# jgsimard/big-dreamer

Measured on AMD Instinct MI355X. Metric: latent transitions/sec (RSSM + imagination) at batch=50 chunk=50 H=15, higher is better.
Workload: dtype f32

## Files before the change

big_dreamer_amd/_cabi.py:

```python
from __future__ import annotations

import ctypes as C
import os

import torch

_HERE = os.path.dirname(os.path.abspath(__file__))
LIB_PATH = os.environ.get("BD_LIB") or os.path.join(_HERE, "libbigdreamer_hip.so")

if not os.path.exists(LIB_PATH):
    raise ImportError(
        f"{LIB_PATH} is missing: the MI355X HIP extension has not been built "
        "(run `python -c 'import __graft_entry__ as g; g.build()'`). There is no CPU fallback.")

lib = C.CDLL(LIB_PATH)

BD_MAX_LAYERS = 6
ACT_NONE, ACT_ELU, ACT_ELU_GRAD = 0, 1, 2
P = C.c_void_p
F32 = C.c_float
I32 = C.c_int


class PackDesc(C.Structure):
    _fields_ = [("src", P), ("dst", P), ("ld", I32), ("N", I32), ("K", I32), ("transpose", I32)]


class Layer(C.Structure):
    _fields_ = [("w", P), ("bias", P), ("N", I32), ("K", I32), ("act", I32), ("save", P)]


class MlpFwdArgs(C.Structure):
    _fields_ = [("M", I32), ("in0", P), ("ld0", I32), ("w0", I32), ("in1", P), ("ld1", I32), ("w1", I32),
                ("n_layers", I32), ("layer", Layer * BD_MAX_LAYERS), ("out", P), ("ldo", I32),
                ("gidx", P), ("gWT", P), ("gD", I32), ("gC", I32)]


class LayerBwd(C.Structure):
    _fields_ = [("wt", P), ("saved", P), ("N", I32), ("K", I32), ("act", I32), ("dpre", P)]


class MlpBwdArgs(C.Structure):
    _fields_ = [("M", I32), ("dout", P), ("lddo", I32), ("dout_scale", F32), ("n_layers", I32),
                ("layer", LayerBwd * BD_MAX_LAYERS), ("din0", P), ("ld0", I32), ("w0", I32),
                ("din1", P), ("ld1", I32), ("w1", I32), ("accumulate", I32)]


BD_RNG_MAX_TENSORS = 6
BD_RNG_NORMAL, BD_RNG_EXPONENTIAL = 0, 1


class RngTensor(C.Structure):
    _fields_ = [("p", P), ("count", C.c_size_t), ("kind", I32), ("stream_id", C.c_uint)]


class RngFillArgs(C.Structure):
    _fields_ = [("n", I32), ("seed", C.c_ulonglong), ("step", C.c_ulonglong), ("t", RngTensor * BD_RNG_MAX_TENSORS)]


class WgradDesc(C.Structure):
    _fields_ = [("dpre", P), ("ldp", I32), ("act1", P), ("lda1", I32), ("M1", I32), ("act2", P), ("lda2", I32),
                ("M", I32), ("N", I32), ("K", I32), ("dW", P), ("ldw", I32), ("db", P),
                ("splits", I32), ("rows_per", I32), ("tiles_n", I32), ("tiles_k", I32), ("block_begin", I32),
                ("red_begin", I32), ("ws_off", C.c_ulonglong),
                ("g_nseg", I32), ("g_seglen", I32), ("g_gh", I32), ("g_gw", I32), ("g_IH", I32), ("g_IW", I32), ("g_C", I32),
                ("g_pad", I32)]


def _ptr_fields(names):
    return [(n, P) for n in names]


class ObserveFwdArgs(C.Structure):
    _fields_ = ([(n, I32) for n in ("T", "B", "Be", "S", "A", "Hd")] + _ptr_fields(
        ["w_embed_s", "w_embed_a", "b_embed", "w_ir", "w_iz", "w_in", "w_hr", "w_hz", "w_hn", "b_ih", "b_hh",
         "w_q1h", "b_q1", "w_q2m", "w_q2s", "b_q2", "init_belief", "init_state", "actions", "nonterm", "pre_emb",
         "eps_post"]) + [("min_std", F32)] + _ptr_fields(
        ["feat", "post_mean", "post_std", "sv_s", "sv_x", "sv_gates", "sv_q"]))


class ObserveBwdArgs(C.Structure):
    _fields_ = ([(n, I32) for n in ("T", "B", "Be", "S", "A", "Hd")] + _ptr_fields(
        ["wt_embed_s", "wt_ir", "wt_iz", "wt_in", "wt_hr", "wt_hz", "wt_hn", "wt_q1h", "wt_q2m", "wt_q2s",
         "init_belief", "nonterm", "eps_post", "feat", "post_std", "sv_x", "sv_gates", "sv_q", "dfeat", "dpost_mean",
         "dpost_std"]) + [("min_std", F32)] + _ptr_fields(
        ["d_embed_pre", "d_gi", "d_gh", "d_q1_pre", "d_q2_out"]))


class ImagineFwdArgs(C.Structure):
    _fields_ = ([(n, I32) for n in ("N", "Hm", "Be", "S", "A", "Hd", "n_samples")] + _ptr_fields(
        ["w_embed_s", "w_embed_a", "b_embed", "w_ir", "w_iz", "w_in", "w_hr", "w_hz", "w_hn", "b_ih", "b_hh", "w_p1",
         "b_p1", "w_p2m", "w_p2s", "b_p2", "w_a0h", "w_a0s"]) + [("w_a", P * 3), ("b_a", P * 4)] + _ptr_fields(
        ["w_a4m", "w_a4s", "b_a4", "start_feat", "eps_action", "eps_entropy", "eps_prior"]) + [
        ("min_std", F32), ("act_raw_init_std", F32), ("act_min_std", F32), ("act_mean_scale", F32)] + _ptr_fields(
        ["feat", "prior_mean", "prior_std", "entropy", "action", "sv_actor", "sv_act_stats", "sv_x", "sv_gates",
         "sv_p"]) + [("sv_actor_stride", C.c_size_t)] + _ptr_fields(["sv_act_us"]) + [("discrete_actions", I32)])


# ... 57 lines not shown
                ("OH", I32), ("OW", I32), ("osy", I32), ("oy0", I32), ("osx", I32), ("ox0", I32), ("ldo", I32),
                ("act", I32), ("fuse_cq", I32), ("aux", P)]


_SIGS = {
    "bd_last_error": (C.c_char_p, []),
    "bd_version": (I32, []),
    "bd_packed_floats": (C.c_size_t, [I32, I32]),
    "bd_pack_weights": (I32, [P, I32, P]),
    "bd_mlp_forward": (I32, [C.POINTER(MlpFwdArgs), P]),
    "bd_mlp_backward": (I32, [C.POINTER(MlpBwdArgs), P]),
    "bd_mlp_set_tall": (I32, [I32]),
    "bd_wgrad_ws_floats": (C.c_size_t, [I32, I32, I32]),
    "bd_wgrad": (I32, [P, I32, P, I32, I32, I32, I32, P, I32, P, I32, P, C.c_size_t, P]),
    "bd_wgrad_plan": (I32, [C.POINTER(WgradDesc), I32, C.POINTER(I32), C.POINTER(I32), C.POINTER(C.c_size_t)]),
    "bd_wgrad_grouped": (I32, [P, I32, I32, I32, P, P]),
    "bd_wgrad_grouped_phase": (I32, [P, I32, I32, I32, P, I32, P]),
    "bd_observe_forward": (I32, [C.POINTER(ObserveFwdArgs), P]),
    "bd_observe_backward": (I32, [C.POINTER(ObserveBwdArgs), P]),
    "bd_observe_cluster_size": (I32, [I32, I32]),
    "bd_observe_cluster_ws_floats": (C.c_size_t, [I32, I32]),
    "bd_observe_forward_cluster": (I32, [C.POINTER(ObserveFwdArgs), P, C.c_size_t, P]),
    "bd_observe_backward_cluster": (I32, [C.POINTER(ObserveBwdArgs), P, C.c_size_t, P]),
    "bd_observe_cluster_status": (I32, [P, I32, P]),
    "bd_observe_cluster_err_offset": (C.c_size_t, [I32]),
    "bd_observe_cluster_set_spin_limit": (I32, [C.c_uint]),
    "bd_observe_cluster_set_ksplit": (I32, [I32]),
    "bd_gauss_head_forward": (I32, [P, P, I32, I32, F32, P, P, P, P]),
    "bd_gauss_head_backward": (I32, [P, P, P, P, P, I32, I32, P, P]),
    "bd_observe_cat_forward": (I32, [C.POINTER(ObserveCatFwdArgs), P]),
    "bd_observe_cat_backward": (I32, [C.POINTER(ObserveCatBwdArgs), P]),
    "bd_observe_cat_cluster_size": (I32, [I32, I32, I32, I32, I32]),
    "bd_observe_cat_cluster_ws_floats": (C.c_size_t, [I32, I32, I32, I32, I32]),
    "bd_observe_cat_forward_cluster": (I32, [C.POINTER(ObserveCatFwdArgs), I32, P, C.c_size_t, P]),
    "bd_observe_cat_backward_cluster": (I32, [C.POINTER(ObserveCatBwdArgs), I32, P, C.c_size_t, P]),
    "bd_imagine_cat_forward": (I32, [C.POINTER(ImagineCatFwdArgs), P]),
    "bd_imagine_cat_backward": (I32, [C.POINTER(ImagineCatBwdArgs), P]),
    "bd_imagine_forward": (I32, [C.POINTER(ImagineFwdArgs), P]),
    "bd_imagine_forward_scan": (I32, [C.POINTER(ImagineFwdArgs), P]),
    "bd_actor_entropy": (I32, [P, P, P, I32, I32, I32, I32, P]),
    "bd_imagine_backward": (I32, [C.POINTER(ImagineBwdArgs), P]),
    "bd_lambda_return_forward": (I32, [P, P, I32, I32, F32, F32, P, P]),
    "bd_rng_fill": (I32, [C.POINTER(RngFillArgs), P]),
    "bd_philox4x32_10": (I32, [C.POINTER(C.c_uint), C.POINTER(C.c_uint), C.POINTER(C.c_uint)]),
    "bd_actor_entropy_rng": (I32, [C.c_ulonglong, C.c_ulonglong, C.c_uint, P, P, I32, I32, I32, I32, P]),
    "bd_gemm_nt": (I32, [P, I32, P, I32, P, I32, I32, I32, I32, I32, P]),
    "bd_categorical_head_forward": (I32, [P, P, I32, I32, I32, P, P, P]),
    "bd_categorical_head_backward": (I32, [P, P, I32, I32, I32, P, P]),
    "bd_kl_categorical_forward": (I32, [P, P, I32, I32, I32, F32, I32, P, I32, P, P]),
    "bd_kl_categorical_backward": (I32, [P, P, I32, I32, I32, F32, F32, F32, F32, P, I32, P, P, P]),
    "bd_plan_rollout": (I32, [C.POINTER(PlanArgs), P]),
    "bd_cem_refit": (I32, [P, I32, P, I32, I32, I32, I32, I32, P, P, P]),
    "bd_lambda_return_backward": (I32, [P, F32, I32, I32, F32, F32, P, P, P]),
    "bd_actor_reinforce": (I32, [P, P, P, P, P, P, P, I32, I32, I32, F32, F32, F32, I32, P, P, I32, P, P]),
    "bd_actor_reinforce_cat": (I32, [P, P, P, P, P, P, I32, I32, I32, F32, F32, F32, I32, P, P, I32, P, P]),
    "bd_normal_nll": (I32, [P, I32, P, I32, I32, I32, F32, P, I32, P, I32, P, P]),
    "bd_bernoulli_nll": (I32, [P, P, C.c_size_t, F32, P, P, I32, P, P]),
    "bd_kl_forward": (I32, [P, P, P, P, I32, I32, F32, I32, P, I32, P, P]),
    "bd_kl_backward": (I32, [P, P, P, P, I32, I32, F32, F32, F32, F32, P, I32, P, P, P, P, P]),
    "bd_sum": (I32, [P, C.c_size_t, P, I32, P, P]),
    "bd_sumsq": (I32, [P, C.c_size_t, P, I32, P, P]),
    "bd_adam_step": (I32, [P, P, P, P, C.c_size_t, F32, F32, F32, F32, F32, I32, F32, P, I32, P]),
    "bd_polyak": (I32, [P, P, C.c_size_t, F32, P]),
    "bd_replay_gather": (I32, [P, P, I32, I32, P, P]),
    "bd_replay_gather_pixels": (I32, [P, P, I32, I32, I32, P, P, P]),
    "bd_replay_gather_pixels_rng": (I32, [P, P, I32, I32, I32, C.c_ulonglong, C.c_ulonglong, P, P]),
    "bd_reduce_ws_floats": (C.c_size_t, []),
    "bd_conv_gemm": (I32, [C.POINTER(ConvArgs), P]),
    "bd_conv_thin_forward": (I32, [P, I32, I32, I32, I32, I32, P, I32, P, I32, P, P, P]),
    "bd_conv_pack_class": (I32, [P, P, I32, I32, I32, I32, I32, I32, I32, P]),
    "bd_conv_pack_fused": (I32, [P, P, I32, I32, I32, P]),
    "bd_elu_backward": (I32, [P, P, C.c_size_t, P]),
    "bd_image_layout": (I32, [P, P, I32, I32, I32, I32, P]),
    "bd_colsum_ws_floats": (C.c_size_t, [I32]),
    "bd_colsum": (I32, [P, C.c_size_t, I32, P, P, P]),
}

for _name, (_res, _args) in _SIGS.items():
    _fn = getattr(lib, _name)
    _fn.restype = _res
    _fn.argtypes = _args

EXPORTED = tuple(_SIGS)


def check(rc: int) -> None:
    if rc != 0:
        raise RuntimeError("bigdreamer_hip: " + lib.bd_last_error().decode())


def ptr(t) -> int:
    if t is None:
        return None
    if not (t.dtype in (torch.float32, torch.int64, torch.uint8) and t.is_cuda):
        raise TypeError("expected a CUDA fp32/int64/uint8 tensor")
    if not (t.is_contiguous() or (t.dim() == 2 and t.stride(1) == 1 and t.stride(0) >= t.shape[1])):
        raise ValueError(f"non-contiguous tensor (shape {tuple(t.shape)}, strides {t.stride()}) passed to a HIP kernel: "
                         "call .contiguous() first")
    return t.data_ptr()


def stream() -> int:
    return torch.cuda.current_stream().cuda_stream


def packed_floats(N: int, K: int) -> int:
# ... 2 lines not shown
```

big_dreamer_amd/engine.py:

```python
from __future__ import annotations

import collections.abc
import ctypes as C
import math
import os
import weakref
from typing import Dict, List, Optional, Tuple

import numpy as np
import torch

from . import _cabi as cabi
from .parallel import DataParallel
from .synth import DENSE_LAYERS, MODEL_MODULES, Dims, model_modules, param_shapes

lib = cabi.lib
ptr = cabi.ptr

DEFAULT_HP = dict(
    kl_balance=0.8, kl_loss_weight=0.1, free_nats=3.0, grad_clip_norm=100.0, discount=0.995, disclam=0.95,
    model_learning_rate=2e-4, actor_learning_rate=4e-5, value_learning_rate=1e-4, adam_epsilon=1e-5,
    weight_decay=1e-6, entropy_weight=1e-5, polyak_avg=1.0, min_std_dev=0.1, discount_weight=5.0,
    gradient_mixing=-1,
)
# ... 208 lines not shown

class DreamerEngine:
    def __init__(self, dims: Dims, hp: Optional[dict] = None, device="cuda", params: Optional[dict] = None,
                 world_size: int = 1, process_group=None, phase_groups: Optional[dict] = None):
        self.d = dims
        self.pixel = bool(dims.pixel)
        self.hp = dict(DEFAULT_HP)
        if hp:
            self.hp.update({k: v for k, v in hp.items() if k in self.hp})
        self.hp["gradient_mixing"] = check_gradient_mixing(self.hp["gradient_mixing"])
        self.dev = torch.device(device)
        assert self.dev.type == "cuda", "the HIP path needs a GPU (there is no CPU fallback)"
        self.world_size = world_size
        self.pg = process_group
        rehearsal = os.environ.get("BD_FORCE_DP", "0") == "1" and torch.distributed.is_initialized()
        if (phase_groups is None and (world_size > 1 or rehearsal) and os.environ.get("BD_PHASE_GROUPS", "1") != "0"
                and torch.distributed.get_backend(process_group) == "nccl"):
            phase_groups = DataParallel.make_phase_groups("nccl", process_group)
        self.dp = DataParallel(world_size, torch.distributed.get_rank(process_group) if world_size > 1 else 0,
                               process_group, phase_groups)
        if (world_size > 1 or rehearsal) and torch.distributed.get_backend(process_group) == "nccl":
            self.dp.force = self.dp.force or rehearsal
            tiny = torch.zeros(4, dtype=torch.float32, device=self.dev)
            for g in (None, "model", "actor", "critic"):
                self.dp.allreduce_sum_(tiny, g)
            torch.cuda.synchronize(self.dev)
        d = dims
        shapes = param_shapes(d)
        self.groups = {
            "model": ParamGroup([(m, n, s) for m in model_modules(d) for n, s in shapes[m]], self.dev,
                                conv_storage=self.pixel),
            "actor": ParamGroup([("actor", n, s) for n, s in shapes["actor"]], self.dev),
            "critic": ParamGroup([("critic", n, s) for n, s in shapes["critic"]], self.dev),
            "critic_target": ParamGroup([("critic_target", n, s) for n, s in shapes["critic"]], self.dev, False),
        }
        self._mod_group = {m: "model" for m in model_modules(d)}
        self._mod_group.update(actor="actor", critic="critic", critic_target="critic_target")
        if params is not None:
            self.load_params(params)
        self.scalars = torch.zeros(N_SLOTS, dtype=torch.float32, device=self.dev)
        self.red_ws = torch.zeros(int(lib.bd_reduce_ws_floats()), dtype=torch.float32, device=self.dev)
        self._wgrad_ws = torch.zeros(1, dtype=torch.float32, device=self.dev)
        self._wgrad_ws_side = torch.zeros(1, dtype=torch.float32, device=self.dev)
        self._wgrad_ws_early = torch.zeros(1, dtype=torch.float32, device=self.dev)
        self.red_ws_side = torch.zeros(int(lib.bd_reduce_ws_floats()), dtype=torch.float32, device=self.dev)
        self._wbatch = {"model": WgradBatch(self, "model"), "model_early": WgradBatch(self, "model_early", "_wgrad_ws_early"),
                        "actor": WgradBatch(self, "actor", "_wgrad_ws_bh"),
                        "critic": WgradBatch(self, "critic", "_wgrad_ws_side")}
        self.overlap_critic = os.environ.get("BD_OVERLAP_CRITIC", "0") == "1"
        self._side = _engine_stream(self.dev, "side", int(os.environ.get("BD_SIDE_PRIO", "0")))
        self._s_heads = _engine_stream(self.dev, "heads", -1)
        self.img_split = os.environ.get("BD_IMG_SPLIT", "0") == "1"
        self._img_split_rows = 0
        self._s_early = _engine_stream(self.dev, "early", int(os.environ.get("BD_EARLY_PRIO", "0")))
        self.pipeline = os.environ.get("BD_PIPELINE", "1") != "0"
        self._s_wm = _engine_stream(self.dev, "wm", int(os.environ.get("BD_WM_PRIO", "-1")))
        bh_prio = int(os.environ.get("BD_BH_PRIO", "0" if self.pixel else "-1"))
        self._s_bh = _engine_stream(self.dev, "bh", bh_prio)
        self._ev_bh_wm_free: Optional[torch.cuda.Event] = None
        self._ev_bh_done: List[Optional[torch.cuda.Event]] = [None, None]
        self._ev_cr_done: List[Optional[torch.cuda.Event]] = [None, None]
        shared_comm = not all(g in self.dp.groups for g in ("model", "actor", "critic"))
        self.defer_opt = (world_size > 1 and shared_comm) or os.environ.get("BD_DEFER_OPT", "0") == "1"
        if os.environ.get("BD_FORCE_DP", "0") == "1" and torch.distributed.is_initialized():
            self.dp.force = True
            self.defer_opt = shared_comm or os.environ.get("BD_DEFER_OPT", "0") == "1"
        if (world_size > 1 or self.dp.force) and torch.cuda.current_stream(self.dev) == torch.cuda.default_stream(self.dev):
            self._main_stream = _engine_stream(self.dev, "main", 0)
            torch.cuda.set_stream(self._main_stream)
        self._pending_opt: List[tuple] = []
        self._opt_over: Dict[str, dict] = {}
        self._rng_seed: Optional[int] = None
        self._rng_step = {"wm": 0, "bh": 0}
        self._rng_entropy_step = 0
        self._log_ring: List[_LogRecord] = []
        self._log_i = 0
        self._cur_rec: Optional[_LogRecord] = None
        self._wm_done_hist: List[torch.cuda.Event] = []
        self._parity = 0
        self._wgrad_ws_bh = torch.zeros(1, dtype=torch.float32, device=self.dev)
        self.red_ws_bh = torch.zeros(int(lib.bd_reduce_ws_floats()), dtype=torch.float32, device=self.dev)
        self._buf: Dict[str, torch.Tensor] = {}
        self.host_ahead = int(os.environ.get("BD_HOST_AHEAD", "2"))
        self._bh_hist: List["torch.cuda.Event"] = []
        self.use_obs_cluster = os.environ.get("BD_OBS_CLUSTER", "1") != "0"
        self._obs_ws: Optional[torch.Tensor] = None
        self._obs_err_off: Optional[int] = None
        self._timers_on, self._timer_every, self._timer_tick = False, 1, 0
        self._timer_events: Dict[str, List[Tuple[torch.cuda.Event, torch.cuda.Event]]] = {}
        self._build_pack_tables()
        self.conv = None
        if self.pixel:
            from .conv_stack import ConvStacks
            self.conv = ConvStacks(self)
        for g in ("model", "actor", "critic", "critic_target"):
            self.pack(g)

    class _Span:

        def __init__(self, eng, name):
            self.eng, self.name = eng, name

        def __enter__(self):
            self.on = self.eng._timers_on and self.eng._timer_tick % self.eng._timer_every == 0
            if self.on:
                self.e0 = torch.cuda.Event(enable_timing=True)
# ... 951 lines not shown
                ws_c = self._cluster_ws(B)
                cabi.check(lib.bd_observe_backward_cluster(C.byref(b), ptr(ws_c), ws_c.numel(), st))
            else:
                cabi.check(lib.bd_observe_backward(C.byref(b), st))

    def _dynamics_tail(self, batch, emb, obs_t, feat, init_belief, actions, d_e, d_gi, d_gh, d_q1, d_q2, d_p_hid, d_p_out,
                       p_hid, rw_dpre, rw_acts, om_dpre, om_acts, N, B, F) -> None:
        d, hp = self.d, self.hp
        HO = d.head_out
        if self.pixel:
            d_emb = self.buf("d_emb", N, d.E)
            self.mlp_backward(N, d_q1, d.Hd, [("q1e", None, d.Hd, d.E, cabi.ACT_NONE)], [None], [None], din0=d_emb, ld0=d.E,
                              w0=d.E)
            with self.span("encoder_bwd"):
                self.conv.backward_encoder(d_emb, self._wbatch["model"])
        else:
            enc_layers = self._dense_spec("encoder", "enc", d.O, d.E) + [("q1e", None, d.Hd, d.E, cabi.ACT_NONE)]
            enc_acts = [self._buf[f"enc_act{l}"] for l in range(DENSE_LAYERS)]
            enc_dpre = [self.buf(f"enc_dpre{l}", N, d.Hd) for l in range(DENSE_LAYERS)] + [self.buf("d_emb", N, d.E)]
            self.mlp_backward(N, d_q1, d.Hd, enc_layers, enc_acts + [None, None], enc_dpre + [None])

        Gt = lambda n: self.G("transition_model", n)
        wb = self._wbatch["model"]
        wb.add(d_gi, 3 * d.Be, self._buf["sv_x"], d.Be, N, 3 * d.Be, d.Be, Gt("rnn.weight_ih"), d.Be, Gt("rnn.bias_ih"))
        wb.add(d_gh, 3 * d.Be, init_belief, d.Be, N, 3 * d.Be, d.Be, Gt("rnn.weight_hh"), d.Be, Gt("rnn.bias_hh"),
               act2=feat, lda2=F, M1=B)
        gWe = Gt("fc_embed_state_action.0.weight")
        wb.add(d_e, d.Be, self._buf["sv_s"], d.S, N, d.Be, d.S, gWe, d.S + d.A, Gt("fc_embed_state_action.0.bias"))
        wb.add(d_e, d.Be, actions[:-1], d.A, N, d.Be, d.A, gWe[:, d.S:], d.S + d.A)
        wb.add(d_p_hid, d.Hd, feat, F, N, d.Hd, d.Be, Gt("belief_prior.model.0.weight"), d.Be, Gt("belief_prior.model.0.bias"))
        wb.add(d_p_out, HO, p_hid, d.Hd, N, HO, d.Hd, Gt("belief_prior.model.2.weight"), d.Hd,
               Gt("belief_prior.model.2.bias"))
        gWq1 = Gt("belief_posterior.model.0.weight")
        wb.add(d_q1, d.Hd, feat, F, N, d.Hd, d.Be, gWq1, d.Be + d.E, Gt("belief_posterior.model.0.bias"))
        wb.add(d_q1, d.Hd, emb, d.E, N, d.Hd, d.E, gWq1[:, d.Be:], d.Be + d.E)
        wb.add(d_q2, HO, self._buf["sv_q"], d.Hd, N, HO, d.Hd, Gt("belief_posterior.model.2.weight"), d.Hd,
               Gt("belief_posterior.model.2.bias"))
        dense_sizes = lambda i, o: [i] + [d.Hd] * DENSE_LAYERS + [o]
        self._dense_wgrads(wb, "reward_model", N, rw_dpre, feat, F, rw_acts, dense_sizes(F, 1))
        if self._dc_wgrad is not None:
            self._dense_wgrads(wb, "discount_model", N, self._dc_wgrad[0], feat, F, self._dc_wgrad[1], dense_sizes(F, 1))
        if not self.pixel:
            self._dense_wgrads(wb, "observation_model", N, om_dpre, feat, F, om_acts, dense_sizes(F, d.O))
            self._dense_wgrads(wb, "encoder", N, enc_dpre, obs_t, d.O, enc_acts, dense_sizes(d.O, d.E))
        with self.span("wgrad_model"):
            wb.run()
        if self.pixel:
            torch.cuda.current_stream().wait_stream(self._s_early)
        if self.pipeline and self._ev_bh_wm_free is not None:
            torch.cuda.current_stream().wait_event(self._ev_bh_wm_free)
        with self.span("opt_model"):
            self.optimizer_step("model", SLOT_GN_MODEL, hp["model_learning_rate"])

    def _behaviour_phase(self, feat: torch.Tensor, noise: Dict[str, torch.Tensor], T: int, B: int,
                         red_ws: torch.Tensor, par: Optional[int]) -> None:
        d, hp, pk = self.d, self.hp, self.pk
        Hm = d.Hm
        N = T * B
        Mi = Hm * N
        F = d.Be + d.S
        st = cabi.stream()
        sc, ws = ptr(self.scalars), ptr(red_ws)
        sum_form = int(hp["kl_balance"] == -1)
        ptag = "" if par is None else f"p{par}_"
        if par is not None and self._ev_cr_done[par] is not None:
            torch.cuda.current_stream().wait_event(self._ev_cr_done[par])
        mix = self._mix
        dyn = mix is None or mix > 0
        start_sidx = self._buf[ptag + "sidx"] if d.categorical else None
        act_us = self.buf("act_us", Mi, 2 * d.A) if mix is not None and not d.discrete_actions else None
        ifeat, ent, act = self.imagine(feat, N, Hm, noise, feat_tag=ptag, split=self.img_split, start_sidx=start_sidx,
                                       rec_saves=dyn, act_us=act_us)
        r0 = self._img_split_rows
        isidx = self._buf[ptag + "isidx"] if d.categorical else None
        with self.span("img_heads_fwd"):
            if not r0:
                r_out, r_acts, r_layers = self.dense_forward("reward_model", "rew", "ir", ifeat, F, Mi, 1, sidx=isidx)
                v_out, v_acts, v_layers = self.dense_forward("critic_target", "tgt", "iv", ifeat, F, Mi, 1, sidx=isidx)
            else:
                with torch.cuda.stream(self._s_heads):
                    self._s_heads.wait_event(self._ev_img_half)
                    self.dense_forward("reward_model", "rew", "ir", ifeat, F, Mi, 1, rows=(0, r0))
                    self.dense_forward("critic_target", "tgt", "iv", ifeat, F, Mi, 1, rows=(0, r0))
                r_out, r_acts, r_layers = self.dense_forward("reward_model", "rew", "ir", ifeat, F, Mi, 1, rows=(r0, Mi))
                v_out, v_acts, v_layers = self.dense_forward("critic_target", "tgt", "iv", ifeat, F, Mi, 1, rows=(r0, Mi))
                torch.cuda.current_stream().wait_stream(self._s_heads)
        returns = self.buf(ptag + "returns", Mi)
        cabi.check(lib.bd_lambda_return_forward(ptr(r_out), ptr(v_out), Hm, N, hp["discount"], hp["disclam"], ptr(returns), st))
        cabi.check(lib.bd_sum(ptr(returns), Mi, sc, SLOT_RET, ws, st))
        cabi.check(lib.bd_sum(ptr(ent), Mi, sc, SLOT_ENT, ws, st))
        inv_mi = self.dp.mean_grad_scale(Mi)
        wts = dret = None
        if d.use_discount:
            dl, _, _ = self.dense_forward("discount_model", "dsc", "idc", ifeat, F, Mi, 1, sidx=isidx)
            arr = hp["discount"] * torch.round(torch.sigmoid(dl.view(Hm, N)))
            arr[:, 0] = 1.0
            wts = self.buf(ptag + "disc_w", Mi)
            wts.view(Hm, N).copy_(torch.cumprod(arr, 0))
            ew_ = hp["entropy_weight"] if hp["entropy_weight"] != -1 else 0.0
            if mix is None:
                self.scalars[SLOT_WOBJ] = (wts * (returns + ew_ * ent)).sum()
                dret = self.buf("dret_w", Mi)
                torch.mul(wts, -inv_mi, out=dret)
            else:
                self.scalars[SLOT_WOBJ] = (wts * (mix * returns + ew_ * ent)).sum()
                if dyn:
                    dret = self.buf("dret_w", Mi)
                    torch.mul(wts, -mix * inv_mi, out=dret)
        if par is not None:
            ev_ret = torch.cuda.Event()
            ev_ret.record(torch.cuda.current_stream())
            with torch.cuda.stream(self._side):
                self._side.wait_event(ev_ret)
                self._critic_phase(ifeat, returns, Mi, F, inv_mi, self.red_ws_side, isidx, wts)
                self._ev_cr_done[par] = torch.cuda.Event()
                self._ev_cr_done[par].record(self._side)
        elif self.overlap_critic:
            self._side.wait_stream(torch.cuda.current_stream())
            with torch.cuda.stream(self._side):
                self._critic_phase(ifeat, returns, Mi, F, inv_mi, self.red_ws_side, isidx, wts)
        dentropy = -hp["entropy_weight"] * inv_mi if hp["entropy_weight"] != -1 else 0.0
        d_apre, d_aout = self.buf("d_actor_pre", DENSE_LAYERS, Mi, d.Hd), self.buf("d_actor_out", Mi, d.actor_out)
        sv_actor = self._buf["sv_actor"]
        actor_chain = os.environ.get("BD_ACTOR_BWD_CHAIN", "1") == "1" or mix is not None or d.discrete_actions
        if dyn:
            d_r, d_v = self.buf("d_ir_out", Mi), self.buf("d_iv_out", Mi)
            dconst = -inv_mi if mix is None else -mix * inv_mi
            cabi.check(lib.bd_lambda_return_backward(ptr(dret), dconst, Hm, N, hp["discount"], hp["disclam"], ptr(d_r),
                                                     ptr(d_v), st))
            difeat = self.buf("difeat", Mi, F)
            with self.span("img_heads_bwd"):
                self.mlp_backward(Mi, d_r, 1, r_layers, r_acts + [None], None, din0=difeat, ld0=F, w0=F)
                self.mlp_backward(Mi, d_v, 1, v_layers, v_acts + [None], None, din0=difeat, ld0=F, w0=F, accumulate=True)
            if d.categorical:
                c = cabi.ImagineCatBwdArgs()
                c.N, c.Hm, c.Be, c.D, c.C, c.A, c.Hd = N, Hm, d.Be, d.cat_D, d.cat_C, d.A, d.Hd
                c.wt_p2 = ptr(pk["p2.T"])
                c.prior_logits = ptr(self._buf["iprior_logits"])
            else:
                c = cabi.ImagineBwdArgs()
                c.N, c.Hm, c.Be, c.S, c.A, c.Hd = N, Hm, d.Be, d.S, d.A, d.Hd
                c.wt_p2m, c.wt_p2s = ptr(pk["p2m.T"]), ptr(pk["p2s.T"])
                c.prior_std, c.eps_prior, c.min_std = ptr(self._buf["iprior_std"]), ptr(noise["img_prior"]), hp["min_std_dev"]
            c.wt_embed_s, c.wt_embed_a = ptr(pk["embed_s.T"]), ptr(pk["embed_a.T"])
            c.wt_ir, c.wt_iz, c.wt_in = ptr(pk["ir.T"]), ptr(pk["iz.T"]), ptr(pk["in.T"])
            c.wt_hr, c.wt_hz, c.wt_hn = ptr(pk["hr.T"]), ptr(pk["hz.T"]), ptr(pk["hn.T"])
            c.wt_p1 = ptr(pk["p1.T"])
            for l in range(1, DENSE_LAYERS):
                c.wt_a[l - 1] = ptr(pk[f"a{l}.T"])
            if d.discrete_actions:
                c.wt_a4m, c.discrete_actions = ptr(pk["a4.T"]), 1
            else:
                c.wt_a4m, c.wt_a4s = ptr(pk["a4m.T"]), ptr(pk["a4s.T"])
            c.start_feat, c.feat, c.action = ptr(feat), ptr(ifeat), ptr(act)
            c.eps_action = ptr(noise["action"])
            c.sv_actor, c.sv_act_stats = ptr(sv_actor), ptr(self._buf["sv_act_stats"])
            c.sv_x, c.sv_gates, c.sv_p = ptr(self._buf["isv_x"]), ptr(self._buf["isv_gates"]), ptr(self._buf["isv_p"])
            c.dfeat = ptr(difeat)
            c.dentropy = dentropy
            c.d_actor_pre, c.d_actor_out = (None if actor_chain else ptr(d_apre)), ptr(d_aout)
            c.ent_weight = ptr(wts)
            with self.span("imagine_bwd"):
                cabi.check((lib.bd_imagine_cat_backward if d.categorical else lib.bd_imagine_backward)(C.byref(c), st))
        if mix is not None:
            with self.span("actor_reinforce"):
                b0, _, _ = self.dense_forward("critic_target", "tgt", "ib0", feat, F, N, 1, sidx=start_sidx)
                if d.discrete_actions:
                    cabi.check(lib.bd_actor_reinforce_cat(ptr(act), ptr(self._buf["sv_act_stats"]), ptr(returns), ptr(b0),
                                                          ptr(v_out), ptr(wts), Hm, N, d.A, mix, inv_mi, dentropy,
                                                          int(not dyn), ptr(d_aout), sc, SLOT_RF, ws, st))
                else:
                    cabi.check(lib.bd_actor_reinforce(ptr(noise["action"]), ptr(act_us), ptr(self._buf["sv_act_stats"]),
                                                      ptr(returns), ptr(b0), ptr(v_out), ptr(wts), Hm, N, d.A, mix, inv_mi,
                                                      dentropy, int(not dyn), ptr(d_aout), sc, SLOT_RF, ws, st))
        if actor_chain:
            a_layers = [("a0h", None, d.Hd, F, cabi.ACT_ELU)] + [(f"a{l}", None, d.Hd, d.Hd, cabi.ACT_ELU)
                                                                  for l in range(1, DENSE_LAYERS)] + \
                       [("a4", None, d.actor_out, d.Hd, cabi.ACT_NONE)]
            with self.span("actor_hidden_bwd"):
                self.mlp_backward(Mi, d_aout, d.actor_out, a_layers, [sv_actor[l] for l in range(DENSE_LAYERS)] + [None],
                                  [d_apre[l] for l in range(DENSE_LAYERS)] + [None])
        if self.pipeline:
            self._ev_bh_wm_free = torch.cuda.Event()
            self._ev_bh_wm_free.record(torch.cuda.current_stream())
        Ga = lambda n: self.G("actor", n)
        wa = self._wbatch["actor"]
# ... 88 lines not shown
```

include/bigdreamer_hip.h:

```cpp
#ifndef BIGDREAMER_HIP_H
#define BIGDREAMER_HIP_H

#include <stddef.h>
#include <stdint.h>

#ifdef __cplusplus
extern "C" {
#endif

#define BD_MAX_LAYERS 6
#define BD_ACT_NONE 0
#define BD_ACT_ELU 1
#define BD_ACT_ELU_GRAD 2

const char* bd_last_error(void);
int bd_version(void);

typedef struct {
    const float* src;
    float* dst;
    int ld;
    int N, K;
    int transpose;
} bd_pack_desc;
// ... 158 lines not shown
    const float* w_a0h; const float* w_a0s; const float* w_a[3]; const float* b_a[4];
    const float* w_a4m; const float* w_a4s; const float* b_a4;
    const float* start_feat;
    const float* eps_action;
    const float* eps_entropy;
    const float* eps_prior;
    float min_std, act_raw_init_std, act_min_std, act_mean_scale;
    float* feat;
    float* prior_mean;
    float* prior_std;
    float* entropy;
    float* action;
    float* sv_actor;
    float* sv_act_stats;
    float* sv_x;
    float* sv_gates;
    float* sv_p;
    size_t sv_actor_stride;
    float* sv_act_us;
    int discrete_actions;
} bd_imagine_fwd_args;
int bd_imagine_forward(const bd_imagine_fwd_args* a, void* stream);
int bd_imagine_forward_scan(const bd_imagine_fwd_args* a, void* stream);
int bd_actor_entropy(const float* eps_entropy, float* act_stats, float* entropy, int Hm, int N, int A, int n_samples,
                     void* stream);

typedef struct {
    int N, Hm, Be, S, A, Hd;
    const float* wt_embed_s; const float* wt_embed_a;
    const float* wt_ir; const float* wt_iz; const float* wt_in;
    const float* wt_hr; const float* wt_hz; const float* wt_hn;
    const float* wt_p1; const float* wt_p2m; const float* wt_p2s;
    const float* wt_a[3];
    const float* wt_a4m; const float* wt_a4s;
    const float* start_feat; const float* feat; const float* prior_std; const float* action;
    const float* eps_action; const float* eps_prior;
    const float* sv_actor; const float* sv_act_stats; const float* sv_x; const float* sv_gates;
    const float* sv_p;
    float min_std;
    const float* dfeat;
    float dentropy;
    float* d_actor_pre;
    float* d_actor_out;
    const float* ent_weight;
    int discrete_actions;
} bd_imagine_bwd_args;
int bd_imagine_backward(const bd_imagine_bwd_args* a, void* stream);

int bd_lambda_return_forward(const float* reward, const float* value, int Hm, int N, float discount,
                             float lambda_, float* returns, void* stream);
int bd_lambda_return_backward(const float* dreturns, float dret_const, int Hm, int N, float discount,
                              float lambda_, float* dreward, float* dvalue, void* stream);

int bd_actor_reinforce(const float* eps_action, const float* act_us, const float* act_stats, const float* returns,
                       const float* base0, const float* value, const float* weight, int Hm, int N, int A, float rho,
                       float grad_scale, float dentropy, int write, float* d_actor_out, float* scalars, int slot, float* ws,
                       void* stream);
int bd_actor_reinforce_cat(const float* action, const float* act_stats, const float* returns, const float* base0,
                           const float* value, const float* weight, int Hm, int N, int A, float rho, float grad_scale,
                           float dentropy, int write, float* d_actor_out, float* scalars, int slot, float* ws,
                           void* stream);

#define BD_RNG_MAX_TENSORS 6
#define BD_RNG_NORMAL 0
#define BD_RNG_EXPONENTIAL 1
typedef struct {
    int n;
    unsigned long long seed;
    unsigned long long step;
    struct {
        float* p;
        size_t count;
        int kind;
        unsigned stream_id;
    } t[BD_RNG_MAX_TENSORS];
} bd_rng_fill_args;
int bd_rng_fill(const bd_rng_fill_args* a, void* stream);
int bd_philox4x32_10(const unsigned* ctr4, const unsigned* key2, unsigned* out4);
int bd_actor_entropy_rng(unsigned long long seed, unsigned long long step, unsigned stream_id, float* act_stats,
                         float* entropy, int Hm, int N, int A, int n_samples, void* stream);

int bd_gemm_nt(const float* A, int lda, const float* B, int ldb, float* C, int ldc, int M, int N, int K, int accumulate,
               void* stream);

int bd_categorical_head_forward(const float* logits, const float* q_noise, int rows, int D, int C, float* state,
                                float* probs, void* stream);
int bd_categorical_head_backward(const float* dstate, const float* probs, int rows, int D, int C, float* dlogits,
                                 void* stream);
int bd_kl_categorical_forward(const float* post_logits, const float* prior_logits, int rows, int D, int C, float free_nats,
                              int sum_form, float* scalars, int slot, float* ws, void* stream);
int bd_kl_categorical_backward(const float* post_logits, const float* prior_logits, int rows, int D, int C, float free_nats,
                               float kl_balance, float weight, float inv_count, const float* scalars, int slot,
                               float* dpost, float* dprior, void* stream);

typedef struct {
    int T, B, Be, D, C, A, Hd;
    const float* w_embed_sT;
    const float* w_embed_a; const float* b_embed;
    const float* w_ir; const float* w_iz; const float* w_in;
    const float* w_hr; const float* w_hz; const float* w_hn;
    const float* b_ih; const float* b_hh;
    const float* w_q1h; const float* b_q1;
    const float* w_q2; const float* b_q2;
    const float* init_belief;
    const float* init_state;
    const float* actions;
// ... 135 lines not shown
```

Before: 12.95 million.

## Fuse imagination reward and value heads forward+backward into one kernel

Adds a HIP kernel that, per row tile, runs the reward and target-critic MLP heads forward, computes their output gradients, backpropagates through both heads, and writes the summed input gradient, all while keeping activations in LDS. The engine computes the lambda-return backward before the head forward so the output gradients exist in time, then calls the fused kernel instead of separate dense forward and mlp_backward launches. This is meant to cut kernel launches and global-memory round-trips of saved activations, at the cost of per-block register and LDS pressure and a restriction to non-categorical models with supported Hd. The return-gradient calculation is reordered so it no longer depends on the forward outputs.

```diff
diff --git a/big_dreamer_amd/_cabi.py b/big_dreamer_amd/_cabi.py
--- a/big_dreamer_amd/_cabi.py
+++ b/big_dreamer_amd/_cabi.py
@@ -44,6 +44,18 @@
     _fields_ = [("M", I32), ("dout", P), ("lddo", I32), ("dout_scale", F32), ("n_layers", I32),
                 ("layer", LayerBwd * BD_MAX_LAYERS), ("din0", P), ("ld0", I32), ("w0", I32),
                 ("din1", P), ("ld1", I32), ("w1", I32), ("accumulate", I32)]
+
+
+BD_HEAD_HIDDEN = 4
+
+
+class ImgHead(C.Structure):
+    _fields_ = [("w", P * BD_HEAD_HIDDEN), ("wt", P * BD_HEAD_HIDDEN), ("b", P * BD_HEAD_HIDDEN),
+                ("w_out", P), ("b_out", P), ("dout", P), ("out", P)]
+
+
+class ImgHeadsArgs(C.Structure):
+    _fields_ = [("M", I32), ("F", I32), ("Hd", I32), ("x", P), ("head", ImgHead * 2), ("dx", P)]
 
 
 BD_RNG_MAX_TENSORS = 6
@@ -207,6 +219,8 @@
     "bd_plan_rollout": (I32, [C.POINTER(PlanArgs), P]),
     "bd_cem_refit": (I32, [P, I32, P, I32, I32, I32, I32, I32, P, P, P]),
     "bd_lambda_return_backward": (I32, [P, F32, I32, I32, F32, F32, P, P, P]),
+    "bd_img_heads_supported": (I32, [I32, I32]),
+    "bd_img_heads_fwd_bwd": (I32, [C.POINTER(ImgHeadsArgs), P]),
     "bd_actor_reinforce": (I32, [P, P, P, P, P, P, P, I32, I32, I32, F32, F32, F32, I32, P, P, I32, P, P]),
     "bd_actor_reinforce_cat": (I32, [P, P, P, P, P, P, I32, I32, I32, F32, F32, F32, I32, P, P, I32, P, P]),
     "bd_normal_nll": (I32, [P, I32, P, I32, I32, I32, F32, P, I32, P, I32, P, P]),
diff --git a/big_dreamer_amd/csrc/heads.hip b/big_dreamer_amd/csrc/heads.hip
--- /dev/null
+++ b/big_dreamer_amd/csrc/heads.hip
@@ -0,0 +1,193 @@
+#include "bd_device.h"
+#include "bd_host.h"
+#include <stdlib.h>
+
+namespace bd {
+
+constexpr int kHeadHidden = BD_HEAD_HIDDEN;
+
+template <int RT, class F>
+__device__ __forceinline__ void tall_map(int N, const TallAcc<RT>& t, const TallAcc<RT>& u, TallAcc<RT>& o, F&& f) {
+    const int wave = bd_wave(bd_tid());
+    const int Nb = (N + 15) >> 4, per = Nb / kWaves;
+#pragma unroll
+    for (int i = 0; i < kTallMaxPer; ++i)
+        if (i < per) {
+#pragma unroll
+            for (int rt = 0; rt < RT; ++rt) o.main[i][rt] = f(rt, wave + i * kWaves, t.main[i][rt], u.main[i][rt]);
+        }
+    int lrt = 0, lnb = 0;
+    if (tall_left_pair(Nb, RT, wave, lrt, lnb)) o.left = f(lrt, lnb, t.left, u.left);
+}
+
+template <int RT>
+__device__ __forceinline__ void img_store(float* img, int Nb, int rt, int nb, floatx4 v) {
+    *reinterpret_cast<floatx4*>(img + ((rt * Nb + nb) * 64 + (bd_tid() & 63)) * 4) = v;
+}
+
+template <int RT, class KA>
+__device__ __forceinline__ void head_fwd_bwd(KA ka, int h, const float* xim, float* img, int KbF, int Hd,
+                                             int row0, int M, TallAcc<RT>& d0) {
+    const auto& H = ka->head[h];
+    const int Nb = cdiv(Hd, 16);
+    const int lane = bd_tid() & 63, m = lane & 15;
+    TallAcc<RT> sv[kHeadHidden];
+#pragma unroll
+    for (int l = 0; l < kHeadHidden; ++l) {
+        const Seg seg[1] = {{l == 0 ? xim : img, H.w[l], l == 0 ? KbF : Nb}};
+        TallAcc<RT> t;
+        tall_sweep<RT, 1>(seg, H.b[l], Hd, t);
+        lds_barrier();
+        tall_map<RT>(Hd, t, t, sv[l], [&](int rt, int nb, floatx4 acc, floatx4) {
+            floatx4 v;
+#pragma unroll
+            for (int r = 0; r < 4; ++r) v[r] = elu(acc[r]);
+            img_store<RT>(img, Nb, rt, nb, v);
+            return v;
+        });
+        lds_barrier();
+    }
+    {
+        constexpr int kRows = 16 * RT, TPR = kThreads / kRows;
+        static_assert(kThreads % kRows == 0 && TPR <= 64 && (TPR & (TPR - 1)) == 0, "threads per row");
+        const int tid = bd_tid(), row = tid / TPR, part = tid - row * TPR;
+        const int rt = row >> 4, mr = row & 15, n4 = cdiv(Hd, 4);
+        const float* base = img + rt * Nb * kFragFloats;
+        float s = 0.f;
+        for (int c = part; c < n4; c += TPR) {
+            const floatx4 v = *reinterpret_cast<const floatx4*>(base + ((c >> 2) * 64 + (c & 3) * 16 + mr) * 4);
+#pragma unroll
+            for (int r = 0; r < 4; ++r)
+                if (4 * c + r < Hd) s += v[r] * H.w_out[4 * c + r];
+        }
+#pragma unroll
+        for (int o = TPR / 2; o > 0; o >>= 1) s += __shfl_xor(s, o, TPR);
+        const int grow = row0 + row;
+        if (part == 0 && grow < M) H.out[grow] = s + H.b_out[0];
+    }
+    lds_barrier();
+    {
+        TallAcc<RT> t;
+        tall_map<RT>(Hd, sv[kHeadHidden - 1], sv[kHeadHidden - 1], t, [&](int rt, int nb, floatx4 a, floatx4) {
+            const int grow = row0 + rt * 16 + m;
+            const float d = grow < M ? H.dout[grow] : 0.f;
+            const floatx4 w = tall_bias(H.w_out, Hd, nb, lane);
+            floatx4 v;
+#pragma unroll
+            for (int r = 0; r < 4; ++r) v[r] = d * w[r] * elu_grad_from_out(a[r]);
+            img_store<RT>(img, Nb, rt, nb, v);
+            return v;
+        });
+        lds_barrier();
+    }
+#pragma unroll
+    for (int l = kHeadHidden - 1; l >= 1; --l) {
+        const Seg seg[1] = {{img, H.wt[l], Nb}};
+        TallAcc<RT> t;
+        tall_sweep<RT, 1>(seg, nullptr, Hd, t);
+        if (l > 1) lds_barrier();
+        tall_map<RT>(Hd, t, sv[l - 1], l > 1 ? t : d0, [&](int rt, int nb, floatx4 acc, floatx4 a) {
+            const bool in = row0 + rt * 16 + m < M;
+            const int col0 = nb * 16 + 4 * (lane >> 4);
+            floatx4 v = floatx4{0.f, 0.f, 0.f, 0.f};
+#pragma unroll
+            for (int r = 0; r < 4; ++r)
+                if (in && col0 + r < Hd) v[r] = acc[r] * elu_grad_from_out(a[r]);
+            if (l > 1) img_store<RT>(img, Nb, rt, nb, v);
+            return v;
+        });
+        if (l > 1) lds_barrier();
+    }
+}
+
+template <int RT>
+__global__ __launch_bounds__(kThreads) __attribute__((amdgpu_waves_per_eu(4 - RT, 4 - RT))) void img_heads_kernel(bd_img_heads_args a) {
+    extern __shared__ __attribute__((aligned(16))) float smem[];
+    const int KbF = cdiv(a.F, 16), Nb = cdiv(a.Hd, 16);
+    float* xim = smem;
+    float* img = smem + (size_t)RT * (KbF > Nb ? KbF : Nb) * kFragFloats;
+    const int row0 = blockIdx.x * 16 * RT;
+    if (tile_pairs_ok(a.x, a.F, a.F, nullptr, 0))
+        load_tile_concat_pairs<RT>(xim, KbF, row0, a.M, a.x, a.F, a.F, nullptr, 0, 0);
+    else
+        load_tile_concat<RT>(xim, KbF, row0, a.M, a.x, a.F, a.F, nullptr, 0, 0);
+    lds_barrier();
+    BD_KARGS(bd_img_heads_args, ka);
+    TallAcc<RT> d0r, d0v;
+#pragma unroll 1
+    for (int h = 0; h < 2; ++h) {
+        BD_KARGS_FRESH(ka);
+        TallAcc<RT> d0;
+        head_fwd_bwd<RT>(ka, h, xim, img, KbF, a.Hd, row0, a.M, d0);
+        if (h == 0) d0r = d0;
+        else d0v = d0;
+    }
+    lds_barrier();
+    tall_foreach2<RT>(a.Hd, d0r, d0v, [&](int rt, int nb, floatx4 r, floatx4 v) {
+        img_store<RT>(xim, Nb, rt, nb, r);
+        img_store<RT>(img, Nb, rt, nb, v);
+    });
+    lds_barrier();
+    const Seg segs[2] = {{xim, a.head[0].wt[0], Nb}, {img, a.head[1].wt[0], Nb}};
+    const bool rows_full = row0 + 16 * RT <= a.M;
+    tile_linear_g<RT, 2>(segs, nullptr, a.F, [&](int rt, int nb, floatx4 acc) {
+        const int ln = bd_tid() & 63, col = nb * 16 + (ln & 15);
+        const unsigned r0 = (unsigned)(row0 + rt * 16 + 4 * (ln >> 4));
+        if (col >= a.F) return;
+        float* __restrict__ p = a.dx + (r0 * (unsigned)a.F + (unsigned)col);
+#pragma unroll
+        for (int r = 0; r < 4; ++r)
+            if (rows_full || (int)r0 + r < a.M) p[r * (unsigned)a.F] = acc[r];
+    });
+}
+
+static int heads_rt(int Hd) {
+    static const char* force = getenv("BD_HEADS_RT");
+    const bool two = !(force && atoi(force) == 1) && tall_shape_ok(Hd, 2);
+    return two ? 2 : (tall_shape_ok(Hd, 1) ? 1 : 0);
+}
+
+static size_t heads_lds(int RT, int F, int Hd) {
+    const int KbF = cdiv(F, 16), Nb = cdiv(Hd, 16);
+    return (size_t)RT * ((KbF > Nb ? KbF : Nb) + Nb) * kFragFloats * sizeof(float);
+}
+
+}
+
+extern "C" {
+
+int bd_img_heads_supported(int F, int Hd) {
+    using namespace bd;
+    if (F <= 0 || Hd <= 0) return 0;
+    const int rt = heads_rt(Hd);
+    return rt > 0 && heads_lds(rt, F, Hd) <= (size_t)kMaxLds;
+}
+
+int bd_img_heads_fwd_bwd(const bd_img_heads_args* a, void* stream) {
+    using namespace bd;
+    BD_REQUIRE(a && a->M > 0 && a->x && a->dx, "bd_img_heads_fwd_bwd: bad M / x / dx");
+    BD_REQUIRE(bd_img_heads_supported(a->F, a->Hd), "bd_img_heads_fwd_bwd: F=%d, Hd=%d not covered (Hd <= 240 in "
+               "column blocks the waves can balance, LDS <= %d B)", a->F, a->Hd, kMaxLds);
+    BD_REQUIRE((size_t)a->M * (size_t)a->F < ((size_t)1 << 31), "bd_img_heads_fwd_bwd: M*F=%zu needs 64-bit offsets",
+               (size_t)a->M * (size_t)a->F);
+    for (int h = 0; h < 2; ++h) {
+        const bd_img_head& H = a->head[h];
+        bool ok = H.w_out && H.b_out && H.dout && H.out;
+        for (int l = 0; l < BD_HEAD_HIDDEN; ++l) ok = ok && H.w[l] && H.wt[l] && H.b[l];
+        BD_REQUIRE(ok, "bd_img_heads_fwd_bwd: head %d is missing an operand", h);
+    }
+    const int rt = heads_rt(a->Hd);
+    const size_t lds = heads_lds(rt, a->F, a->Hd);
+    const dim3 grid(cdiv(a->M, 16 * rt));
+    if (rt == 2) {
+        if (lds > 64 * 1024 && allow_big_lds(img_heads_kernel<2>)) return -1;
+        hipLaunchKernelGGL(img_heads_kernel<2>, grid, dim3(kThreads), lds, (hipStream_t)stream, *a);
+    } else {
+        if (lds > 64 * 1024 && allow_big_lds(img_heads_kernel<1>)) return -1;
+        hipLaunchKernelGGL(img_heads_kernel<1>, grid, dim3(kThreads), lds, (hipStream_t)stream, *a);
+    }
+    BD_CHECK_LAUNCH("bd_img_heads_fwd_bwd");
+    return 0;
+}
+
+}
diff --git a/big_dreamer_amd/engine.py b/big_dreamer_amd/engine.py
--- a/big_dreamer_amd/engine.py
+++ b/big_dreamer_amd/engine.py
@@ -284,6 +284,8 @@
         self._s_heads = _engine_stream(self.dev, "heads", -1)
         self.img_split = os.environ.get("BD_IMG_SPLIT", "0") == "1"
         self._img_split_rows = 0
+        self.heads_fused = (os.environ.get("BD_HEADS_FUSED", "1") != "0" and not self.d.categorical
+                            and bool(lib.bd_img_heads_supported(self.d.Be + self.d.S, self.d.Hd)))
         self._s_early = _engine_stream(self.dev, "early", int(os.environ.get("BD_EARLY_PRIO", "0")))
         self.pipeline = os.environ.get("BD_PIPELINE", "1") != "0"
         self._s_wm = _engine_stream(self.dev, "wm", int(os.environ.get("BD_WM_PRIO", "-1")))
@@ -1341,6 +1343,21 @@
         with self.span("opt_model"):
             self.optimizer_step("model", SLOT_GN_MODEL, hp["model_learning_rate"])
 
+    def img_heads_fused(self, M: int, x, d_r, d_v, r_out, v_out, dx) -> None:
+        d = self.d
+        a = cabi.ImgHeadsArgs()
+        a.M, a.F, a.Hd, a.x, a.dx = M, d.Be + d.S, d.Hd, ptr(x), ptr(dx)
+        for h, (mod, prefix, dout, out) in enumerate((("reward_model", "rew", d_r, r_out),
+                                                      ("critic_target", "tgt", d_v, v_out))):
+            H = a.head[h]
+            for l in range(DENSE_LAYERS):
+                H.w[l], H.wt[l] = ptr(self.pk[f"{prefix}{l}"]), ptr(self.pk[f"{prefix}{l}.T"])
+                H.b[l] = ptr(self.W(mod, f"model.{2 * l}.bias"))
+            H.w_out = ptr(self.W(mod, f"model.{2 * DENSE_LAYERS}.weight"))
+            H.b_out = ptr(self.W(mod, f"model.{2 * DENSE_LAYERS}.bias"))
+            H.dout, H.out = ptr(dout), ptr(out)
+        cabi.check(lib.bd_img_heads_fwd_bwd(C.byref(a), cabi.stream()))
+
     def _behaviour_phase(self, feat: torch.Tensor, noise: Dict[str, torch.Tensor], T: int, B: int,
                          red_ws: torch.Tensor, par: Optional[int]) -> None:
         d, hp, pk = self.d, self.hp, self.pk
@@ -1362,22 +1379,6 @@
                                        rec_saves=dyn, act_us=act_us)
         r0 = self._img_split_rows
         isidx = self._buf[ptag + "isidx"] if d.categorical else None
-        with self.span("img_heads_fwd"):
-            if not r0:
-                r_out, r_acts, r_layers = self.dense_forward("reward_model", "rew", "ir", ifeat, F, Mi, 1, sidx=isidx)
-                v_out, v_acts, v_layers = self.dense_forward("critic_target", "tgt", "iv", ifeat, F, Mi, 1, sidx=isidx)
-            else:
-                with torch.cuda.stream(self._s_heads):
-                    self._s_heads.wait_event(self._ev_img_half)
-                    self.dense_forward("reward_model", "rew", "ir", ifeat, F, Mi, 1, rows=(0, r0))
-                    self.dense_forward("critic_target", "tgt", "iv", ifeat, F, Mi, 1, rows=(0, r0))
-                r_out, r_acts, r_layers = self.dense_forward("reward_model", "rew", "ir", ifeat, F, Mi, 1, rows=(r0, Mi))
-                v_out, v_acts, v_layers = self.dense_forward("critic_target", "tgt", "iv", ifeat, F, Mi, 1, rows=(r0, Mi))
-                torch.cuda.current_stream().wait_stream(self._s_heads)
-        returns = self.buf(ptag + "returns", Mi)
-        cabi.check(lib.bd_lambda_return_forward(ptr(r_out), ptr(v_out), Hm, N, hp["discount"], hp["disclam"], ptr(returns), st))
-        cabi.check(lib.bd_sum(ptr(returns), Mi, sc, SLOT_RET, ws, st))
-        cabi.check(lib.bd_sum(ptr(ent), Mi, sc, SLOT_ENT, ws, st))
         inv_mi = self.dp.mean_grad_scale(Mi)
         wts = dret = None
         if d.use_discount:
@@ -1386,16 +1387,48 @@
             arr[:, 0] = 1.0
             wts = self.buf(ptag + "disc_w", Mi)
             wts.view(Hm, N).copy_(torch.cumprod(arr, 0))
+            if mix is None:
+                dret = self.buf("dret_w", Mi)
+                torch.mul(wts, -inv_mi, out=dret)
+            elif dyn:
+                dret = self.buf("dret_w", Mi)
+                torch.mul(wts, -mix * inv_mi, out=dret)
+        fused = dyn and self.heads_fused
+        if dyn:
+            d_r, d_v = self.buf("d_ir_out", Mi), self.buf("d_iv_out", Mi)
+            dconst = -inv_mi if mix is None else -mix * inv_mi
+            difeat = self.buf("difeat", Mi, F)
+        if fused:
+            cabi.check(lib.bd_lambda_return_backward(ptr(dret), dconst, Hm, N, hp["discount"], hp["disclam"], ptr(d_r),
+                                                     ptr(d_v), st))
+            r_out, v_out = self.buf("ir_out", Mi, 1), self.buf("iv_out", Mi, 1)
+            with self.span("img_heads_bwd"):
+                self.img_heads_fused(Mi, ifeat, d_r, d_v, r_out, v_out, difeat)
+        else:
+            with self.span("img_heads_fwd"):
+                if not r0:
+                    r_out, r_acts, r_layers = self.dense_forward("reward_model", "rew", "ir", ifeat, F, Mi, 1, sidx=isidx)
+                    v_out, v_acts, v_layers = self.dense_forward("critic_target", "tgt", "iv", ifeat, F, Mi, 1, sidx=isidx)
+                else:
+                    with torch.cuda.stream(self._s_heads):
+                        self._s_heads.wait_event(self._ev_img_half)
+                        self.dense_forward("reward_model", "rew", "ir", ifeat, F, Mi, 1, rows=(0, r0))
+                        self.dense_forward("critic_target", "tgt", "iv", ifeat, F, Mi, 1, rows=(0, r0))
+                    r_out, r_acts, r_layers = self.dense_forward("reward_model", "rew", "ir", ifeat, F, Mi, 1,
+                                                                 rows=(r0, Mi))
+                    v_out, v_acts, v_layers = self.dense_forward("critic_target", "tgt", "iv", ifeat, F, Mi, 1,
+                                                                 rows=(r0, Mi))
+                    torch.cuda.current_stream().wait_stream(self._s_heads)
+        returns = self.buf(ptag + "returns", Mi)
+        cabi.check(lib.bd_lambda_return_forward(ptr(r_out), ptr(v_out), Hm, N, hp["discount"], hp["disclam"], ptr(returns), st))
+        cabi.check(lib.bd_sum(ptr(returns), Mi, sc, SLOT_RET, ws, st))
+        cabi.check(lib.bd_sum(ptr(ent), Mi, sc, SLOT_ENT, ws, st))
+        if d.use_discount:
             ew_ = hp["entropy_weight"] if hp["entropy_weight"] != -1 else 0.0
             if mix is None:
                 self.scalars[SLOT_WOBJ] = (wts * (returns + ew_ * ent)).sum()
-                dret = self.buf("dret_w", Mi)
-                torch.mul(wts, -inv_mi, out=dret)
             else:
                 self.scalars[SLOT_WOBJ] = (wts * (mix * returns + ew_ * ent)).sum()
-                if dyn:
-                    dret = self.buf("dret_w", Mi)
-                    torch.mul(wts, -mix * inv_mi, out=dret)
         if par is not None:
             ev_ret = torch.cuda.Event()
             ev_ret.record(torch.cuda.current_stream())
@@ -1413,14 +1446,13 @@
         sv_actor = self._buf["sv_actor"]
         actor_chain = os.environ.get("BD_ACTOR_BWD_CHAIN", "1") == "1" or mix is not None or d.discrete_actions
         if dyn:
-            d_r, d_v = self.buf("d_ir_out", Mi), self.buf("d_iv_out", Mi)
-            dconst = -inv_mi if mix is None else -mix * inv_mi
-            cabi.check(lib.bd_lambda_return_backward(ptr(dret), dconst, Hm, N, hp["discount"], hp["disclam"], ptr(d_r),
-                                                     ptr(d_v), st))
-            difeat = self.buf("difeat", Mi, F)
-            with self.span("img_heads_bwd"):
-                self.mlp_backward(Mi, d_r, 1, r_layers, r_acts + [None], None, din0=difeat, ld0=F, w0=F)
-                self.mlp_backward(Mi, d_v, 1, v_layers, v_acts + [None], None, din0=difeat, ld0=F, w0=F, accumulate=True)
+            if not fused:
+                cabi.check(lib.bd_lambda_return_backward(ptr(dret), dconst, Hm, N, hp["discount"], hp["disclam"],
+                                                         ptr(d_r), ptr(d_v), st))
+                with self.span("img_heads_bwd"):
+                    self.mlp_backward(Mi, d_r, 1, r_layers, r_acts + [None], None, din0=difeat, ld0=F, w0=F)
+                    self.mlp_backward(Mi, d_v, 1, v_layers, v_acts + [None], None, din0=difeat, ld0=F, w0=F,
+                                      accumulate=True)
             if d.categorical:
                 c = cabi.ImagineCatBwdArgs()
                 c.N, c.Hm, c.Be, c.D, c.C, c.A, c.Hd = N, Hm, d.Be, d.cat_D, d.cat_C, d.A, d.Hd
diff --git a/include/bigdreamer_hip.h b/include/bigdreamer_hip.h
--- a/include/bigdreamer_hip.h
+++ b/include/bigdreamer_hip.h
@@ -234,6 +234,25 @@
 int bd_lambda_return_backward(const float* dreturns, float dret_const, int Hm, int N, float discount,
                               float lambda_, float* dreward, float* dvalue, void* stream);
 
+#define BD_HEAD_HIDDEN 4
+typedef struct {
+    const float* w[BD_HEAD_HIDDEN];
+    const float* wt[BD_HEAD_HIDDEN];
+    const float* b[BD_HEAD_HIDDEN];
+    const float* w_out;
+    const float* b_out;
+    const float* dout;
+    float* out;
+} bd_img_head;
+typedef struct {
+    int M, F, Hd;
+    const float* x;
+    bd_img_head head[2];
+    float* dx;
+} bd_img_heads_args;
+int bd_img_heads_supported(int F, int Hd);
+int bd_img_heads_fwd_bwd(const bd_img_heads_args* a, void* stream);
+
 int bd_actor_reinforce(const float* eps_action, const float* act_us, const float* act_stats, const float* returns,
                        const float* base0, const float* value, const float* weight, int Hm, int N, int A, float rho,
                        float grad_scale, float dentropy, int write, float* d_actor_out, float* scalars, int slot, float* ws,
```

Result: faster. 13.28 million (median of 6 runs) (+2.5%).
